# harrisonvanderbyl/rwkv-cpp-accelerated

Measured on AMD Instinct MI355X. Metric: tokens/sec single-stream RWKV-4 uint8 greedy decode, higher is better.
Workload: dtype u8 weights x 23-bit fixed-point activations, exact 32-bit integer accumulate (tile form: v_mfma_i32_16x16x64_i8 on signed limbs; row form: v_dot4_u32_u8 on the VALU); f32/f64 epilogues, f64 state; 1 GPU; RWKV-4-Raven-7B uint8 single-stream greedy decode (L=32, D=4096, V=50277), 32-token prompt then 1885-token continuation, device-resident state; parallelism=1 GPU

## Files before the change

rwkv-cpp-accelerated_amd/csrc/engine.hip:

```cpp
#include "kernels.hip.h"
#include "tile.hip.h"
#include "seq.hip.h"
#include "sampler.hip.h"
#include "../../include/rwkv_mi355x.h"

#include <dlfcn.h>

#include <algorithm>
#include <atomic>
#include <chrono>
#include <unistd.h>
#include <cstdarg>
#include <cstdio>
#include <cstdlib>
#include <cstring>
#include <map>
#include <string>
#include <tuple>
#include <vector>

using namespace rwkvk;

namespace {

// ... 127 lines not shown
    int seq_rows = SEQ_TM;
    int seq_b = -1;
    int tile = -1;

    float *embed = nullptr;
    double *ln = nullptr, *mixk = nullptr, *mixv = nullptr, *mixr = nullptr, *fmixk = nullptr, *fmixr = nullptr;
    float *kr = nullptr, *vr = nullptr, *rr = nullptr, *o1 = nullptr, *o2 = nullptr, *o3 = nullptr;
    float *attr = nullptr, *atto = nullptr, *fkr = nullptr, *fvr = nullptr, *frr = nullptr;
    float *fko = nullptr, *fvo = nullptr, *fro = nullptr, *headr = nullptr, *heado = nullptr;
    double *uw = nullptr, *ew = nullptr;
    float *siteC[3] = {nullptr, nullptr, nullptr};
    float *siteP[3] = {nullptr, nullptr, nullptr};
    double *siteTC[3] = {nullptr, nullptr, nullptr};
    float *siteMC[3] = {nullptr, nullptr, nullptr};
    float *siteB[3] = {nullptr, nullptr, nullptr};
    double *sitePD[3] = {nullptr, nullptr, nullptr};
    float *sitePF[3] = {nullptr, nullptr, nullptr};
    double *lnstat = nullptr;
    uint8_t *w_kvr = nullptr, *w_att = nullptr, *w_frk = nullptr, *w_fv = nullptr, *w_head = nullptr;
    unsigned *rs_kvr = nullptr, *rs_att = nullptr, *rs_frk = nullptr, *rs_fv = nullptr, *rs_head = nullptr;
    double *state[5] = {nullptr, nullptr, nullptr, nullptr, nullptr};
    double *x = nullptr, *partA = nullptr, *partF = nullptr;
    float *ybuf = nullptr, *hbuf = nullptr, *rgate = nullptr, *logits = nullptr, *blk_val = nullptr, *partMA = nullptr, *partMF = nullptr;
    unsigned *blk_idx = nullptr;
    Ctl *ctl = nullptr;
    Ctl *h_ctl = nullptr;
    unsigned long long *gen = nullptr;
    unsigned long long *pick = nullptr;
    double *ts_part = nullptr;
    float *ts_p = nullptr, *ts_pw = nullptr;
    unsigned *ts_key = nullptr;
    unsigned gen_cap = 0;
    hipGraphExec_t g_fwd = nullptr, g_greedy = nullptr;
    unsigned *herr = nullptr, *d_herr = nullptr;
    unsigned long long *tl = nullptr;
    bool tl_on = false;
    int tl_cls = 3;
    bool seq_ok = false;
    unsigned long long *sq_tokens = nullptr;
    unsigned long long *h_sq_tokens = nullptr;
    hipEvent_t sq_ev[8] = {};
    uint64_t sq_n = 0;
    struct SeqGraphKey { uint64_t la, lb, row0; int buf, n; bool operator<(const SeqGraphKey &o) const { return std::tie(la, lb, row0, buf, n) < std::tie(o.la, o.lb, o.row0, o.buf, o.n); } };
    std::map<SeqGraphKey, hipGraphExec_t> sq_graphs;
    bool seq_graph = true;
    int graphs = 3;
    double *sq_x[4] = {nullptr, nullptr, nullptr, nullptr};
    hipEvent_t xs_ev[2] = {nullptr, nullptr};
    static constexpr int SPLIT_MAX = 4;
    int n_split = 0;
    hipStream_t sp_stream[SPLIT_MAX] = {};
    struct SeqScratch *sp_scratch[SPLIT_MAX] = {};
    hipEvent_t sp_done[SPLIT_MAX][SPLIT_MAX] = {};
    hipEvent_t sp_end = nullptr;
    double *x_in = nullptr;
    struct Pipe *pipe = nullptr;
    bool pipe_prof = false;
    static constexpr size_t HOP_EV = 512;
    hipEvent_t hop_ev[2 * HOP_EV] = {};
    double hop_stats[4] = {0.0, 0.0, 0.0, 0.0};
    Ctl *pipe_ring = nullptr;
    uint64_t pipe_ring_cap = 0;
    double *sq_state = nullptr;
    float *sq_y = nullptr;
    unsigned *sq_img[3] = {nullptr, nullptr, nullptr}, *sq_imgh = nullptr;
    SeqPart *sq_qpart = nullptr, *sq_qparta = nullptr, *sq_qparth = nullptr;
// ... 86 lines not shown
    HIPCHK(hipFuncSetAttribute(reinterpret_cast<const void *>(kernel), hipFuncAttributeMaxDynamicSharedMemorySize, (int)bytes));
    return 0;
}


struct ArgMaker {
    rwkv_ctx *c;
    int D, grid, n_first;
    size_t LD;
    explicit ArgMaker(rwkv_ctx *c_) : c(c_), D((int)c_->D), grid(c_->grid), LD((size_t)c_->L * c_->D) { n_first = grid < 32 ? grid : 32; }
    unsigned long long *tl_of(int k, uint64_t l) const { return (c->tl_on && k == c->tl_cls && l == (c->l0 + c->l1) / 2) ? c->tl : nullptr; }
    SiteStatic site_static(int k, uint64_t ll) const
    {
        const int nv = SITE_NV[k], pw = SITE_PW[k];
        SiteStatic st;
        st.C = c->siteC[k] + (size_t)ll * nv * D; st.P = c->siteP[k] + (size_t)ll * D * pw;
        st.TC = c->siteTC[k] + (size_t)ll * nv; st.maxC = c->siteMC[k] + (size_t)ll * nv;
        st.invD = 1.0 / (double)D; st.invDm1 = 1.0 / (double)(D - 1);
        return st;
    }
    SiteDyn site_dyn(int k, int n_part) const
    {
        SiteDyn dy;
        dy.B = c->siteB[k]; dy.pd = c->sitePD[k]; dy.pf = c->sitePF[k]; dy.lnstat = c->lnstat + 2 * k; dy.n_part = n_part;
        return dy;
    }
    FirstArgs first() const
    {
        FirstArgs fa;
        fa.embed = c->embed; fa.ln = c->ln; fa.x = c->x; fa.x_in = c->x_in ? c->x_in : c->x; fa.st = site_static(0, c->l0); fa.dy = site_dyn(0, n_first);
        fa.sxy = c->state[0] + (size_t)c->l0 * D; fa.slot_stride = LD; fa.ctl = c->ctl; fa.D = D; fa.from_token = c->l0 == 0;
        return fa;
    }
    AttArgs att(uint64_t l) const
    {
        const size_t lo = (size_t)l * D;
        AttArgs aa;
        aa.x = c->x; aa.st = site_static(0, l); aa.dy = site_dyn(0, l == c->l0 ? n_first : grid);
        aa.w = c->w_kvr ? c->w_kvr + (size_t)(l - c->l0) * 3 * D * D : nullptr; aa.rs = c->rs_kvr + (size_t)(l - c->l0) * D * 3;
        aa.uw = c->uw + lo; aa.ew = c->ew + lo;
        aa.r_att = c->attr + lo; aa.o_att = c->atto + lo;
        aa.saa = c->state[1] + lo; aa.sbb = c->state[2] + lo;
        aa.slot_stride = LD; aa.ybuf = c->ybuf; aa.partS = c->partA; aa.partM = c->partMA;
        aa.ctl = c->ctl; aa.D = D; aa.ns = 0; aa.tl = tl_of(1, l); aa.herr = c->d_herr;
        return aa;
    }
    AttOutArgs attout(uint64_t l) const
    {
        const size_t lo = (size_t)l * D;
        AttOutArgs ao;
        ao.w = c->w_att ? c->w_att + (size_t)(l - c->l0) * D * D : nullptr; ao.rs = c->rs_att + (size_t)(l - c->l0) * D; ao.ybuf = c->ybuf; ao.partS = c->partA; ao.partM = c->partMA; ao.n_part = grid;
        ao.x = c->x; ao.lnw = c->ln + (4 * l + 2) * D; ao.lnb = c->ln + (4 * l + 3) * D; ao.lnstat = c->lnstat + 0;
        ao.sxy = c->state[0] + lo; ao.st = site_static(1, l); ao.dy = site_dyn(1, grid); ao.sdd = c->state[4] + lo;
        ao.slot_stride = LD; ao.ctl = c->ctl; ao.D = D; ao.ns = 0; ao.tl = tl_of(2, l); ao.herr = c->d_herr;
        return ao;
    }
    FfnRKArgs frk(uint64_t l) const
    {
        const size_t lo = (size_t)l * D;
        FfnRKArgs fa;
        fa.x = c->x; fa.st = site_static(1, l); fa.dy = site_dyn(1, grid);
        fa.w = c->w_frk ? c->w_frk + (size_t)(l - c->l0) * 5 * D * D : nullptr; fa.rs = c->rs_frk + (size_t)(l - c->l0) * D * 5;
        fa.r_fv = c->fvr + 4 * lo; fa.o_fv = c->fvo + 4 * lo;
        fa.hbuf = c->hbuf; fa.rgate = c->rgate; fa.partS = c->partF; fa.partM = c->partMF; fa.ctl = c->ctl; fa.D = D;
        fa.ns = 0; fa.tl = tl_of(3, l); fa.herr = c->d_herr;
        return fa;
// ... 63 lines not shown
            ta.im.CB = mk.D / c->tile_th; ta.im.bimg = c->t_frk + (size_t)(l - c->l0) * 5 * (size_t)mk.D * mk.D;
            const size_t sm = tile_smem(c, 3);
            TILE_DISPATCH(c, (k_ffn_rk_t<4, 4, 64, 16, 1><<<dim3(grid), dim3(NT), sm, c->stream>>>(ta)),
                          (k_ffn_rk_t<5, 5, 20, 4, 5><<<dim3(grid), dim3(NT), sm, c->stream>>>(ta)),
                          (k_ffn_rk_t<2, 4, 8, 4, 2><<<dim3(grid), dim3(NT), sm, c->stream>>>(ta)));
        }
        else DISPATCH_S(S, k_ffn_rk<S_><<<dim3(grid), dim3(NT), smem_frk(S), c->stream>>>(fa));
    } break;
    case 4: {
        FfnVArgs fv = mk.fv(l);
        if (tile_ok(c, 4)) {
            FfnVTArgs ta;
            ta.a = fv; ta.a.ns = tile_units(c, 4);
            ta.im.CB = mk.D / c->tile_th; ta.im.bimg = c->t_fv + (size_t)(l - c->l0) * 4 * (size_t)mk.D * mk.D;
            const size_t sm = tile_smem(c, 4);
            if (mk.fv_next_att(l))
                TILE_DISPATCH(c, (k_ffnv_t<4, 4, 256, 16, 1, 3><<<dim3(grid), dim3(NT), sm, c->stream>>>(ta)),
                              (k_ffnv_t<5, 5, 80, 4, 5, 3><<<dim3(grid), dim3(NT), sm, c->stream>>>(ta)),
                              (k_ffnv_t<2, 4, 32, 4, 2, 3><<<dim3(grid), dim3(NT), sm, c->stream>>>(ta)));
            else
                TILE_DISPATCH(c, (k_ffnv_t<4, 4, 256, 16, 1, 1><<<dim3(grid), dim3(NT), sm, c->stream>>>(ta)),
                              (k_ffnv_t<5, 5, 80, 4, 5, 1><<<dim3(grid), dim3(NT), sm, c->stream>>>(ta)),
                              (k_ffnv_t<2, 4, 32, 4, 2, 1><<<dim3(grid), dim3(NT), sm, c->stream>>>(ta)));
        }
        else if (mk.fv_next_att(l)) {
            DISPATCH_S(S, k_ffnv<S_, 3><<<dim3(grid), dim3(NT), smem_fv(S), c->stream>>>(fv));
        } else {
            DISPATCH_S(S, k_ffnv<S_, 1><<<dim3(grid), dim3(NT), smem_fv(S), c->stream>>>(fv));
        }
    } break;
    case 5: {
        HeadArgs ha = mk.head();
        DISPATCH_S(S, k_head<S_><<<dim3(grid), dim3(NT), smem_head(S), c->stream>>>(ha));
    } break;
    default:
        k_argmax_finish<<<dim3(1), dim3(64), 0, c->stream>>>(c->blk_val, c->blk_idx, grid, c->ctl, c->gen, c->gen_cap);
    }
}

int device_check(rwkv_ctx *c)
{
    if (!c->herr || *c->herr == 0u) return 0;
    const unsigned code = *c->herr;
    *c->herr = 0u;
    return fail(RWKV_E_DEVICE, "a device-side wait gave up (code %u: an LDS hand-off timed out; is the GPU shared or preempted?) -- "
                               "the results of this call are invalid; RWKV_TILE=0 selects kernels without bounded waits", code);
}

int enqueue_token(rwkv_ctx *c, bool with_argmax, hipEvent_t *ev)
{
    const bool last = c->l1 == c->L;
    int evi = 0;
#define EV() do { if (ev) HIPCHK(hipEventRecord(ev[evi++], c->stream)); } while (0)
    EV();
    launch_class(c, 0, 0);
    for (uint64_t l = c->l0; l < c->l1; l++)
        for (int cls = 1; cls <= 4; cls++) { EV(); launch_class(c, cls, l); }
    EV();
    if (last) launch_class(c, 5, 0);
    EV();
    if (last && with_argmax) launch_class(c, 6, 0);
    EV();
#undef EV
    HIPCHK(hipGetLastError());
    return 0;
}

int build_graph(rwkv_ctx *c, bool with_argmax, hipGraphExec_t *out)
{
    hipGraph_t g = nullptr;
    HIPCHK(hipStreamBeginCapture(c->stream, hipStreamCaptureModeRelaxed));
    int rc = enqueue_token(c, with_argmax, nullptr);
    hipError_t e = hipStreamEndCapture(c->stream, &g);
    if (rc) return rc;
    HIPCHK(e);
    HIPCHK(hipGraphInstantiate(out, g, nullptr, nullptr, 0));
    HIPCHK(hipGraphDestroy(g));
    return 0;
}

int rebuild_graphs(rwkv_ctx *c)
{
    int rc = 0;
    if (c->g_fwd) { (void)hipGraphExecDestroy(c->g_fwd); c->g_fwd = nullptr; rc = build_graph(c, false, &c->g_fwd); if (rc) { c->g_fwd = nullptr; return rc; } }
    if (c->g_greedy) { (void)hipGraphExecDestroy(c->g_greedy); c->g_greedy = nullptr; rc = build_graph(c, true, &c->g_greedy); if (rc) { c->g_greedy = nullptr; return rc; } }
    return 0;
}

int retile(rwkv_ctx *c, Source &src, int slot, uint64_t layer, uint64_t N, uint64_t M, uint8_t *dst,
           int G, int RS, int off, uint8_t *staging)
{
    const uint8_t *dsrc = static_cast<const uint8_t *>(src.device_ptr(slot, layer * N * M));
    if (!dsrc) {
        int rc = src.to_device(slot, layer * N * M, N * M, staging, c->stream);
        if (rc) return rc;
        dsrc = staging;
    }
    dim3 grid((unsigned)((M + 63) / 64), (unsigned)((N + 63) / 64));
    hipLaunchKernelGGL(k_retile, grid, dim3(256), 0, c->stream, dsrc, dst, (int)N, (int)M, G, RS, off);
    HIPCHK(hipGetLastError());
    return 0;
}

template <typename T> int upload(rwkv_ctx *c, Source &src, int slot, T **dst)
{
    const uint64_t n = tensor_elems(slot, c->L, c->D);
    int rc = dalloc(c, dst, n);
    if (rc) return rc;
    return src.to_device(slot, 0, n * sizeof(T), *dst, c->stream);
}

int seq_smem_limits()
{
    int rc = 0;
#define SEQ_ALLOW_P(TAG, NTW, NKB, NVS, DEPTH, MULTI) if (!rc) rc = allow_smem(k_seq_gemm_p<TAG, NTW, NKB, NVS, DEPTH, MULTI>, seq_gemm_p_smem(NKB, NVS, MULTI))
    SEQ_ALLOW_P(0, 3, 8, 3, RWKV_SEQ_DEPTH0, false); SEQ_ALLOW_P(0, 3, 10, 2, 2, false);
    SEQ_ALLOW_P(1, 1, 8, 1, 8, false); SEQ_ALLOW_P(1, 1, 10, 1, 10, false);
    SEQ_ALLOW_P(2, 5, 8, 2, RWKV_SEQ_DEPTH2, false); SEQ_ALLOW_P(2, 4, 10, 2, 2, false);
// ... 260 lines not shown
            if ((rc = dalloc(c, &c->sq_tokens, (size_t)SQ_RING * SEQ_TM))) return rc;
            HIPCHK(hipHostMalloc(reinterpret_cast<void **>(&c->h_sq_tokens), sizeof(unsigned long long) * SQ_RING * SEQ_TM, hipHostMallocDefault));
            for (int r = 0; r < SQ_RING; r++) HIPCHK(hipEventCreateWithFlags(&c->sq_ev[r], hipEventDisableTiming));
            if ((rc = dalloc(c, &c->sq_x[0], (size_t)SEQ_TM * D))) return rc;
            if ((rc = dalloc(c, &c->sq_x[1], (size_t)SEQ_TM * D))) return rc;
            if ((rc = dalloc(c, &c->sq_state, (size_t)D))) return rc;
            if ((rc = dalloc(c, &c->sq_y, (size_t)SEQ_TM * D))) return rc;
            for (int k = 0; k < 3; k++) {
                if ((rc = dalloc(c, &c->sq_img[k], 2 * a_image_bytes(D) / 4))) return rc;
                HIPCHK(hipMemsetAsync(c->sq_img[k], 0, 2 * a_image_bytes(D), c->stream));
            }
            if ((rc = dalloc(c, &c->sq_imgh, 2 * a_image_bytes(4 * D) / 4))) return rc;
            HIPCHK(hipMemsetAsync(c->sq_imgh, 0, 2 * a_image_bytes(4 * D), c->stream));
            if ((rc = dalloc(c, &c->sq_qpart, (size_t)2 * 3 * SEQ_T * SEQ_O))) return rc;
            if ((rc = dalloc(c, &c->sq_qparta, (size_t)2 * SEQ_T * SEQ_O))) return rc;
            if ((rc = dalloc(c, &c->sq_qparth, (size_t)2 * SEQ_T * SEQ_O))) return rc;
            HIPCHK(hipMemsetAsync(c->sq_qpart, 0, sizeof(SeqPart) * 2 * 3 * SEQ_T * SEQ_O, c->stream));
            HIPCHK(hipMemsetAsync(c->sq_qparta, 0, sizeof(SeqPart) * 2 * SEQ_T * SEQ_O, c->stream));
            HIPCHK(hipMemsetAsync(c->sq_qparth, 0, sizeof(SeqPart) * 2 * SEQ_T * SEQ_O, c->stream));
            if ((rc = dalloc(c, &c->sq_stat, (size_t)SEQ_TM * SEQ_O))) return rc;
            {
                const size_t cbd = ((size_t)D + 15) / 16;
                if ((rc = dalloc(c, &c->sq_pk3, (size_t)2 * SEQ_O * 3 * cbd * 512))) return rc;
                if ((rc = dalloc(c, &c->sq_pk5, (size_t)2 * SEQ_O * 5 * cbd * 512))) return rc;
                if ((rc = dalloc(c, &c->sq_pk1, (size_t)2 * SEQ_O * cbd * 512))) return rc;
            }
            c->seq_ok = true;
        }
    }
    HIPCHK(hipStreamSynchronize(c->stream));
    if ((rc = set_smem_limits(c))) return rc;
    if (c->seq_ok && (rc = seq_smem_limits())) return rc;
    if (c->graphs & 1) {
        if ((rc = build_graph(c, false, &c->g_fwd))) return rc;
        if ((rc = build_graph(c, true, &c->g_greedy))) return rc;
    }
    c->loaded = true;
    return 0;
}

struct ChunkPart { uint64_t la, lb; hipStream_t st; const SeqScratch *S; bool no_upload = false; const unsigned long long *dtok = nullptr; };
int upload_chunk_tokens(rwkv_ctx *c, const uint64_t *tokens, int n, int buf, hipStream_t st)
{
    const int slot = (int)(c->sq_n % SQ_RING);
    if (c->sq_n >= SQ_RING) HIPCHK(hipEventSynchronize(c->sq_ev[slot]));
    unsigned long long *h = c->h_sq_tokens + (size_t)slot * SEQ_TM, *d = c->sq_tokens + (size_t)buf * SEQ_TM;
    for (int t = 0; t < n; t++) h[t] = tokens[t];
    HIPCHK(hipMemcpyAsync(d, h, sizeof(unsigned long long) * n, hipMemcpyHostToDevice, st));
    HIPCHK(hipEventRecord(c->sq_ev[slot], st));
    c->sq_n++;
    return 0;
}
int enqueue_chunk(rwkv_ctx *c, const uint64_t *tokens, int n, uint64_t row0, bool par, int buf = 0, const ChunkPart *part = nullptr)
{
    const int D = (int)c->D;
    const uint64_t L = c->L, V = RWKV_VOCAB;
    const uint64_t la = part ? part->la : c->l0, lb = part ? part->lb : c->l1;
    const bool first = c->l0 == 0 && la == c->l0, last = c->l1 == c->L && lb == c->l1;
    hipStream_t st = part ? part->st : c->stream;
    SeqScratch own;
    own.state = c->sq_state; own.y = c->sq_y; own.imgh = c->sq_imgh;
    for (int k = 0; k < 3; k++) own.img[k] = c->sq_img[k];
    own.qpart = c->sq_qpart; own.qparta = c->sq_qparta; own.qparth = c->sq_qparth; own.stat = c->sq_stat;
    own.pk3 = c->sq_pk3; own.pk5 = c->sq_pk5; own.pk1 = c->sq_pk1;
    const SeqScratch &S = part ? *part->S : own;
    double *x = c->sq_x[buf];
    if (first) {
        if (buf < 0 || buf >= SQ_RING) return fail(RWKV_E_ARG, "residual buffer %d out of range", buf);
// ... 286 lines not shown
                const uint64_t *tk = (k == 0 && tokens) ? tokens + t0 : nullptr;
                if (mode == RWKV_MODE_PARRALEL) rc = enqueue_chunk(c, tk, n, t0, true, b, &part);
                else rc = enqueue_pass(c, tk, n, t0, b, part);
                HIPCHK(hipEventRecord(c->sp_done[k][b], st));
            }
        }
        for (int k = 1; k < ns; k++) {
            HIPCHK(hipEventRecord(c->sp_end, c->sp_stream[k]));
            HIPCHK(hipStreamWaitEvent(c->stream, c->sp_end, 0));
        }
        return rc;
    }
    if (rc) return rc;
    for (uint64_t t0 = 0; t0 < T; t0 += CH) {
        const int n = (int)(T - t0 < CH ? T - t0 : CH);
        ChunkPart part{c->l0, c->l1, c->stream, &own};
        if (dtok) part.dtok = dtok + t0;
        if (mode == RWKV_MODE_PARRALEL) rc = enqueue_chunk(c, tokens ? tokens + t0 : nullptr, n, t0, true, 0, &part);
        else rc = enqueue_pass(c, tokens + t0, n, t0, 0, part);
        if (rc) return rc;
    }
    return 0;
}

int begin_call(rwkv_ctx *c)
{
    if (c->herr) *c->herr = 0u;
    return 0;
}

int run_token(rwkv_ctx *c, bool with_argmax)
{
    hipGraphExec_t g = with_argmax ? c->g_greedy : c->g_fwd;
    if (g) { HIPCHK(hipGraphLaunch(g, c->stream)); return 0; }
    return enqueue_token(c, with_argmax, nullptr);
}

const struct { const char *name, *instead; } RETIRED_ENV[] = {
    {"RWKV_RING", "RWKV_TILE (the LDS-ring form of the row-form decode kernels is gone)"},
    {"RWKV_NO_GRAPH", "RWKV_GRAPH=0"},
    {"RWKV_SEQ_GRAPH", "RWKV_GRAPH bit 1"},
    {"RWKV_SEQ_SPLIT", "RWKV_SEQ_STAGES (RWKV_SEQ_SPLIT=0 is RWKV_SEQ_STAGES=1)"},
    {"RWKV_PIPE_LOG", nullptr},
    {"RWKV_SEQ_PIPE", nullptr},
    {"RWKV_SEQ_SMALL", nullptr},
};
void warn_retired_env()
{
    for (const auto &r : RETIRED_ENV)
        if (getenv(r.name))
            fprintf(stderr, "[rwkv_mi355x] %s is retired and ignored%s%s\n", r.name, r.instead ? "; use " : "", r.instead ? r.instead : "");
}

}

extern "C" {

const char *rwkv_last_error(void) { return g_err.c_str(); }

int rwkv_create(rwkv_ctx **out, int device)
{
    if (!out) return fail(RWKV_E_ARG, "out is NULL");
    int n = 0;
    if (hipGetDeviceCount(&n) != hipSuccess || n <= 0)
        return fail(RWKV_E_DEVICE, "no HIP device available (this engine has no CPU fallback)");
    if (device < 0 || device >= n) return fail(RWKV_E_ARG, "device %d out of range (have %d)", device, n);
    HIPCHK(hipSetDevice(device));
// ... 140 lines not shown
    if (T > c->maxT) return fail(RWKV_E_ARG, "n_tokens %llu > max context %llu", (unsigned long long)T, (unsigned long long)c->maxT);
    double *h[5] = {xy, aa, bb, pp, dd};
    HIPCHK(hipSetDevice(c->device));
    if (logits) HIPCHK(hipMemcpyAsync(logits, c->logits, T * RWKV_VOCAB * sizeof(float), hipMemcpyDeviceToHost, c->stream));
    const size_t bytes = T * c->L * c->D * sizeof(double);
    for (int s = 0; s < 5; s++)
        if (h[s]) HIPCHK(hipMemcpyAsync(h[s], c->state[s], bytes, hipMemcpyDeviceToHost, c->stream));
    HIPCHK(hipStreamSynchronize(c->stream));
    return device_check(c);
}

int rwkv_reset_state(rwkv_ctx *c)
{
    if (!c) return fail(RWKV_E_ARG, "NULL ctx");
    if (!c->loaded) return fail(RWKV_E_STATE, "RWKV not loaded");
    HIPCHK(hipSetDevice(c->device));
    for (int s = 0; s < 5; s++)
        HIPCHK(hipMemsetAsync(c->state[s], 0, c->maxT * c->L * c->D * sizeof(double), c->stream));
    HIPCHK(hipStreamSynchronize(c->stream));
    return device_check(c);
}

int rwkv_decode_greedy(rwkv_ctx *c, uint64_t first_token, uint64_t n, uint64_t *out_tokens)
{
    if (!c || !out_tokens) return fail(RWKV_E_ARG, "NULL argument");
    if (!c->loaded) return fail(RWKV_E_STATE, "RWKV not loaded");
    if (c->l0 != 0 || c->l1 != c->L) return fail(RWKV_E_STATE, "needs a whole-model context (a pipeline stage has no embedding / head of its own)");
    if (first_token >= RWKV_VOCAB) return fail(RWKV_E_ARG, "token id out of range");
    if (n == 0 || n > c->gen_cap) return fail(RWKV_E_ARG, "n_tokens must be in 1..%u", c->gen_cap);
    HIPCHK(hipSetDevice(c->device));
    { const int rcp = begin_call(c); if (rcp) return rcp; }
    c->h_ctl[0].token = first_token; c->h_ctl[0].slot = 0; c->h_ctl[0].out_row = 0; c->h_ctl[0].step = 0; c->h_ctl[0].pad = 0;
    HIPCHK(hipMemcpyAsync(c->ctl, &c->h_ctl[0], sizeof(Ctl), hipMemcpyHostToDevice, c->stream));
    for (uint64_t i = 0; i < n; i++) {
        int rc = run_token(c, true);
        if (rc) return rc;
    }
    HIPCHK(hipMemcpyAsync(out_tokens, c->gen, n * sizeof(uint64_t), hipMemcpyDeviceToHost, c->stream));
    HIPCHK(hipStreamSynchronize(c->stream));
    return device_check(c);
}

namespace {
TypicalArgs typical_args(rwkv_ctx *c, float temp, float tau, int flags)
{
    TypicalArgs a{};
    a.recipe = (flags & RWKV_SAMPLE_RECIPE) ? 1 : 0;
    if (a.recipe) a.expo = temp == 1.0f ? 1.0 : 1.0 / (double)temp;
    else { const double e = 1.0 / (double)temp; a.expo = temp == 1.0f ? 1.0 : (e >= 255.0 ? 255.0 : (double)(unsigned char)e); }
    a.logits = c->logits; a.ctl = c->ctl; a.gen = c->gen; a.gen_cap = c->gen_cap;
    a.temp = temp; a.tau = tau; a.ban0 = (flags & RWKV_SAMPLE_BAN0) ? 1 : 0; a.step = -1; a.seeds = nullptr;
    a.pick = c->pick; a.part = c->ts_part; a.p = c->ts_p; a.pw = c->ts_pw; a.key = c->ts_key;
    return a;
}
int enqueue_typical(rwkv_ctx *c, const TypicalArgs &a, unsigned rows)
{
    k_typical_stats<<<dim3(TS_G, rows), dim3(TS_GT), 0, c->stream>>>(a);
    k_typical_keys<<<dim3(TS_G, rows), dim3(TS_GT), 0, c->stream>>>(a);
    k_typical<<<dim3(1, rows), dim3(TS_NT), 0, c->stream>>>(a);
    HIPCHK(hipGetLastError());
    return 0;
}
int launch_typical(rwkv_ctx *c, int row, float temp, float tau, double u, uint64_t seed, bool use_seed, int flags, bool feedback)
{
    TypicalArgs a = typical_args(c, temp, tau, flags);
    a.row = row; a.u = u; a.seed = seed; a.use_seed = use_seed ? 1 : 0; a.feedback = feedback ? 1 : 0;
    return enqueue_typical(c, a, 1);
}
}

// ... 114 lines not shown
int rwkv_decode_batch_greedy(rwkv_ctx *c, const uint64_t *first_tokens, uint64_t n_streams, uint64_t n_steps, uint64_t *out_tokens)
{
    return decode_batch(c, first_tokens, n_streams, n_steps, false, 1.0f, 0.0f, nullptr, 0, out_tokens);
}

int rwkv_decode_batch_typical(rwkv_ctx *c, const uint64_t *first_tokens, uint64_t n_streams, uint64_t n_steps, float temp, float tau,
                              const uint64_t *seeds, int flags, uint64_t *out_tokens)
{
    return decode_batch(c, first_tokens, n_streams, n_steps, true, temp, tau, seeds, flags, out_tokens);
}

int rwkv_state_copy(rwkv_ctx *c, uint64_t dst, uint64_t src)
{
    if (!c) return fail(RWKV_E_ARG, "NULL ctx");
    if (!c->loaded) return fail(RWKV_E_STATE, "RWKV not loaded");
    if (dst >= c->maxT || src >= c->maxT)
        return fail(RWKV_E_ARG, "state slot out of range (dst %llu, src %llu, max context %llu)", (unsigned long long)dst, (unsigned long long)src, (unsigned long long)c->maxT);
    if (dst == src) return 0;
    const size_t n = (size_t)c->L * c->D;
    HIPCHK(hipSetDevice(c->device));
    for (int s = 0; s < 5; s++)
        HIPCHK(hipMemcpyAsync(c->state[s] + dst * n, c->state[s] + src * n, n * sizeof(double), hipMemcpyDeviceToDevice, c->stream));
    HIPCHK(hipStreamSynchronize(c->stream));
    return device_check(c);
}

void rwkv_free(rwkv_ctx *c)
{
    if (!c) return;
    (void)hipSetDevice(c->device);
    if (c->stream) (void)hipStreamSynchronize(c->stream);
    if (c->g_fwd) { (void)hipGraphExecDestroy(c->g_fwd); c->g_fwd = nullptr; }
    if (c->g_greedy) { (void)hipGraphExecDestroy(c->g_greedy); c->g_greedy = nullptr; }
    rwkv_pipe_free(c);
    for (void *p : c->allocs) (void)hipFree(p);
    for (rwkv_ctx::Grown *g : {&c->bd_ids, &c->bd_val, &c->bd_idx, &c->bd_part, &c->bd_p, &c->bd_pw, &c->bd_key}) if (g->p) (void)hipFree(g->p);
    if (c->h_ctl) (void)hipHostFree(c->h_ctl);
    if (c->herr) (void)hipHostFree(c->herr);
    for (auto &e : c->xs_ev) if (e) (void)hipEventDestroy(e);
    for (auto &e : c->hop_ev) if (e) (void)hipEventDestroy(e);
    for (auto &row : c->sp_done) for (auto &e : row) if (e) (void)hipEventDestroy(e);
    if (c->sp_end) (void)hipEventDestroy(c->sp_end);
    for (int k = 1; k < rwkv_ctx::SPLIT_MAX; k++) { if (c->sp_stream[k]) (void)hipStreamDestroy(c->sp_stream[k]); delete c->sp_scratch[k]; }
    for (auto &kv : c->sq_graphs) (void)hipGraphExecDestroy(kv.second);
    c->sq_graphs.clear();
    if (c->h_sq_tokens) (void)hipHostFree(c->h_sq_tokens);
    for (int r = 0; r < SQ_RING; r++) if (c->sq_ev[r]) (void)hipEventDestroy(c->sq_ev[r]);
    if (c->stream) (void)hipStreamDestroy(c->stream);
    delete c;
}

float *rwkv_logits_device(rwkv_ctx *c) { return c ? c->logits : nullptr; }
double *rwkv_state_device(rwkv_ctx *c, int which) { return (c && which >= 0 && which < 5) ? c->state[which] : nullptr; }
void *rwkv_stream(rwkv_ctx *c) { return c ? (void *)c->stream : nullptr; }
int rwkv_abi_version(void) { return RWKV_MI355X_ABI_VERSION; }
uint64_t rwkv_resident_bytes(const rwkv_ctx *c) { return c ? (uint64_t)c->alloc_bytes : 0; }
int rwkv_decode_form(const rwkv_ctx *c) { return c && c->loaded ? (c->tile > 0 ? c->tile : 0) : -1; }

uint64_t rwkv_bytes_per_token(const rwkv_ctx *c)
{
    if (!c) return 0;
    const uint64_t nl = (c->l1 == UINT64_MAX ? c->L : c->l1) - c->l0, D = c->D, V = RWKV_VOCAB;
    return 13 * nl * D * D + (c->l1 == c->L || c->l1 == UINT64_MAX ? V * D : 0) + 168 * nl * D + 40 * D;
}

int rwkv_profile_token(rwkv_ctx *c, uint64_t token, int reps, double *ms, uint64_t *bytes, uint32_t *launches)
// ... 87 lines not shown
{
    if (!c || !out) return fail(RWKV_E_ARG, "NULL argument");
    if (!c->loaded) return fail(RWKV_E_STATE, "RWKV not loaded");
    const size_t n = (size_t)(c->grid > 512 ? c->grid : 512) * NW * 8;
    if (cap < n) return fail(RWKV_E_ARG, "need room for %zu stamps", n);
    HIPCHK(hipSetDevice(c->device));
    { const int rcp = begin_call(c); if (rcp) return rcp; }
    if (!c->tl) { int rc = dalloc(c, &c->tl, n); if (rc) return rc; }
    HIPCHK(hipMemsetAsync(c->tl, 0, n * 8, c->stream));
    c->h_ctl[0].token = token; c->h_ctl[0].slot = 0; c->h_ctl[0].out_row = 0; c->h_ctl[0].step = 0; c->h_ctl[0].pad = 0;
    HIPCHK(hipMemcpyAsync(c->ctl, &c->h_ctl[0], sizeof(Ctl), hipMemcpyHostToDevice, c->stream));
    { const char *e = getenv("RWKV_TL_CLASS"); c->tl_cls = e ? atoi(e) : 3; }
    c->tl_on = true;
    int rc;
    if (c->tl_cls >= 10) {
        if (!c->seq_ok) { c->tl_on = false; return fail(RWKV_E_STATE, "the chunk path is not loaded (max_ctx 1)"); }
        uint64_t toks[SEQ_TM];
        for (int t = 0; t < SEQ_TM; t++) toks[t] = token;
        int rows = SEQ_T;
        if (c->tl_cls >= 20) { c->tl_cls -= 10; if (c->seq_rows > SEQ_T && c->maxT >= (uint64_t)SEQ_TM) rows = SEQ_TM; }
        rc = enqueue_chunk(c, toks, rows, 0, false);
    } else rc = enqueue_token(c, false, nullptr);
    c->tl_on = false;
    if (rc) return rc;
    HIPCHK(hipMemcpyAsync(out, c->tl, n * 8, hipMemcpyDeviceToHost, c->stream));
    HIPCHK(hipStreamSynchronize(c->stream));
    return device_check(c);
}

int rwkv_debug_launch(rwkv_ctx *c, int cls, uint64_t layer, uint64_t token, uint32_t slot)
{
    if (!c) return fail(RWKV_E_ARG, "NULL ctx");
    if (!c->loaded) return fail(RWKV_E_STATE, "RWKV not loaded");
    if (cls < 0 || cls > 6) return fail(RWKV_E_ARG, "kernel class %d out of range (0 first, 1 att, 2 att_out, 3 ffn r+k, 4 ffn_v, 5 head, 6 argmax)", cls);
    if (cls >= 1 && cls <= 4 && (layer < c->l0 || layer >= c->l1)) return fail(RWKV_E_ARG, "layer %llu is not one of this context's", (unsigned long long)layer);
    if (cls >= 5 && c->l1 != c->L) return fail(RWKV_E_STATE, "this context does not hold the head");
    if (slot >= c->maxT) return fail(RWKV_E_ARG, "state slot %u out of range", slot);
    if (c->l0 == 0 && token >= RWKV_VOCAB) return fail(RWKV_E_ARG, "token id out of range");
    HIPCHK(hipSetDevice(c->device));
    { const int rcp = begin_call(c); if (rcp) return rcp; }
    if (cls == 0) {
        c->h_ctl[0].token = token; c->h_ctl[0].slot = slot; c->h_ctl[0].out_row = slot; c->h_ctl[0].step = 0; c->h_ctl[0].pad = 0;
        HIPCHK(hipMemcpyAsync(c->ctl, &c->h_ctl[0], sizeof(Ctl), hipMemcpyHostToDevice, c->stream));
    }
    launch_class(c, cls, layer);
    HIPCHK(hipGetLastError());
    HIPCHK(hipStreamSynchronize(c->stream));
    return device_check(c);
}

namespace {
int debug_buf(rwkv_ctx *c, int which, void **p, size_t *bytes)
{
    const size_t D = (size_t)c->D, G = (size_t)c->grid;
    switch (which) {
    case RWKV_DBG_X: *p = c->x; *bytes = D * 8; break;
    case RWKV_DBG_YBUF: *p = c->ybuf; *bytes = D * 4; break;
    case RWKV_DBG_PART_ATT: *p = c->partA; *bytes = G * 8; break;
    case RWKV_DBG_PMAX_ATT: *p = c->partMA; *bytes = G * 4; break;
    case RWKV_DBG_HBUF: *p = c->hbuf; *bytes = 4 * D * 4; break;
    case RWKV_DBG_RGATE: *p = c->rgate; *bytes = D * 4; break;
    case RWKV_DBG_PART_FFN: *p = c->partF; *bytes = G * 8; break;
    case RWKV_DBG_PMAX_FFN: *p = c->partMF; *bytes = G * 4; break;
    case RWKV_DBG_LNSTAT: *p = c->lnstat; *bytes = 6 * 8; break;
    default: return fail(RWKV_E_ARG, "no such debug buffer: %d", which);
    }
    return 0;
}
}
// ... 587 lines not shown
```

rwkv-cpp-accelerated_amd/csrc/kernels.hip.h:

```cpp
#pragma once
#include <hip/hip_runtime.h>
#include <stdint.h>

namespace rwkvk {

constexpr int NT = 512;
constexpr int NW = NT / 64;
constexpr int RED_BYTES = 1024;
#define RWKV_ARGS_NOW(...) asm volatile("" ::RWKV_ARGS_S(__VA_ARGS__))
#define RWKV_ARGS_S(...) RWKV_ARGS_PICK(__VA_ARGS__, RWKV_A8, RWKV_A7, RWKV_A6, RWKV_A5, RWKV_A4, RWKV_A3, RWKV_A2, RWKV_A1)(__VA_ARGS__)
#define RWKV_ARGS_PICK(a, b, c, d, e, f, g, h, N, ...) N
#define RWKV_A1(a) "s"(a)
#define RWKV_A2(a, ...) "s"(a), RWKV_A1(__VA_ARGS__)
#define RWKV_A3(a, ...) "s"(a), RWKV_A2(__VA_ARGS__)
#define RWKV_A4(a, ...) "s"(a), RWKV_A3(__VA_ARGS__)
#define RWKV_A5(a, ...) "s"(a), RWKV_A4(__VA_ARGS__)
#define RWKV_A6(a, ...) "s"(a), RWKV_A5(__VA_ARGS__)
#define RWKV_A7(a, ...) "s"(a), RWKV_A6(__VA_ARGS__)
#define RWKV_A8(a, ...) "s"(a), RWKV_A7(__VA_ARGS__)
__device__ __forceinline__ int wave_id() { return __builtin_amdgcn_readfirstlane((int)(threadIdx.x >> 6)); }
__device__ __forceinline__ int block_lo(int n) { return (int)(((unsigned)blockIdx.x * (unsigned)n) / gridDim.x); }
__device__ __forceinline__ int block_hi(int n) { return (int)((((unsigned)blockIdx.x + 1u) * (unsigned)n) / gridDim.x); }
constexpr unsigned VOCAB = 50277u;
constexpr float QLIM = 4194000.0f;
// ... 604 lines not shown
    fail = ok ? fail : 3u;
}
__device__ __forceinline__ void ring_report(unsigned fail, unsigned *herr)
{
    if (fail != 0u && herr != nullptr && (threadIdx.x & 63) == 0) __hip_atomic_store(herr, fail, __ATOMIC_RELAXED, __HIP_MEMORY_SCOPE_SYSTEM);
}
#ifndef RWKV_RING_DEPTH
#define RWKV_RING_DEPTH 28
#endif
#ifndef RWKV_RING_PRE
#define RWKV_RING_PRE 8
#endif
#ifndef RWKV_TEST_DROP_GROUP
#define RWKV_TEST_DROP_GROUP 0
#endif
#ifndef RWKV_RING_PRE_DEPTH
#define RWKV_RING_PRE_DEPTH 20
#endif
constexpr int NC = NW - 1;

struct FirstArgs {
    const float *embed;
    const double *ln;
    double *x;
    const double *x_in;
    SiteStatic st;
    SiteDyn dy;
    const double *sxy;
    size_t slot_stride;
    const Ctl *ctl;
    int D;
    int from_token;
};
__global__ __launch_bounds__(NT) void k_first(FirstArgs a)
{
    __shared__ double red[RED_BYTES / 8];
    const int D = a.D;
    const int j0 = block_lo(D), j1 = block_hi(D);
    const size_t so = (size_t)a.ctl->slot * a.slot_stride;
    double mean = 0.0, rstd = 1.0;
    const float *row = a.from_token ? a.embed + (size_t)a.ctl->token * D : nullptr;
    if (a.from_token) {
        double s[2] = {0.0, 0.0};
        for (int j = threadIdx.x; j < D; j += NT) { const double v = (double)row[j]; s[0] += v; s[1] += v * v; }
        block_sum<2>(s, red + RED_STATS);
        mean = s[0] / (double)D;
        rstd = 1.0 / sqrt((s[1] - s[0] * mean) / (double)(D - 1));
        __syncthreads();
    }
    SiteAcc<3> acc;
    acc.clear();
    for (int j = j0 + threadIdx.x; j < j1; j += NT) {
        double x;
        if (a.from_token) { x = a.ln[j] * (((double)row[j] - mean) * rstd) + a.ln[D + j]; a.x[j] = x; }
        else { x = a.x_in[j]; a.x[j] = x; }
        SitePre<3> pre;
        site_prefetch<3>(a.st, j, pre);
        site_emit<3>(pre, a.dy, D, j, x, a.sxy[so + j], acc);
    }
    site_publish<3, 64>(acc, a.dy, red);
}

struct AttArgs {
    const double *x;
    SiteStatic st;
    SiteDyn dy;
    const uint8_t *w;
    const unsigned *rs;
    const double *uw, *ew;
    const float *r_att, *o_att;
    double *saa, *sbb;
    size_t slot_stride;
    float *ybuf;
    double *partS;
    float *partM;
    const Ctl *ctl;
    int D;
    int ns;
    unsigned long long *tl;
    unsigned *herr;
};

__device__ __forceinline__ void att_epilogue(double *saa, double *sbb, float *ybuf, int g, double aa, double bb, double e1, double ek, float v, float r, double ew, float ra, float oa, double &part, float &pmax)
{
    const double vv = (double)v;
    double y = (aa + e1 * vv) / (bb + e1);
    y = (1.0 / (1.0 + (double)expf(-r))) * y;
    saa[g] = (aa + ek * vv) * ew;
    sbb[g] = (bb + ek) * ew;
    const float yf = (float)y;
    const float ys = yf * ra;
    ybuf[g] = ys;
    part += (double)(yf * oa);
    pmax = fmaxf(pmax, fabsf(ys));
// ... 280 lines not shown
        site_prefetch<NVN>(a.st, g, in.pre);
        return in;
    };
    auto epi = [&](int g, const unsigned long long (&T)[4], const FfnVIn<NVN> &in) {
        if (lane == 0)
            ffnv_epilogue<NVN>(a, so, D, g, row_value((T[0] + T[1]) + (T[2] + T[3]), in.rsum, sc) + Sf, in.rg, in.xold, in.lw, in.lb, in.prevn, mean2, rstd2, in.pre, acc);
    };
    u32x4 wA[4][S];
    int gA;
    unsigned *gctr = group_counter(red);
    first_groups(g0, wave, gctr, gA);
    vec_open<4, 4, S, (RWKV_SPLIT & 8) != 0>(a.hbuf, a.partS, a.partM, a.n_part, D, red, xq, wA, base(gA), (size_t)D, Sf, amax, a.tl);
    sc = scale_of(amax);
    stream_groups<4, S, PAT_PER_ROW>(wA, gA, g0, g1, gctr, xq, lane, (size_t)D, chunks, base, pre, epi);
    __syncthreads();
    tl_stamp(a.tl, 6);
    site_publish<NVN, 1>(acc, a.dy, xq);
    tl_stamp(a.tl, 7);
}

struct HeadArgs {
    const double *x;
    SiteStatic st;
    SiteDyn dy;
    const uint8_t *w;
    const unsigned *rs;
    float *logits;
    float *blk_val;
    unsigned *blk_idx;
    const Ctl *ctl;
    int D;
};

__device__ __forceinline__ bool am_better(float v, unsigned i, float best, unsigned besti) { return v > best || (v == best && i < besti); }
__device__ __forceinline__ void am_wave_fold(float &best, unsigned &besti)
{
#pragma unroll
    for (int m = 32; m >= 1; m >>= 1) {
        const float ov = __shfl_xor(best, m, 64);
        const unsigned oi = __shfl_xor(besti, m, 64);
        if (am_better(ov, oi, best, besti)) { best = ov; besti = oi; }
    }
}

template <int R> struct HeadIn { unsigned rsr[R]; int row0, shift; };
template <int S, int R = RWKV_HEAD_R>
__global__ __launch_bounds__(NT) void k_head(HeadArgs a)
{
    extern __shared__ __attribute__((aligned(16))) unsigned char smem[];
    constexpr int XVD = xvd<S>();
    double *red = reinterpret_cast<double *>(smem);
    unsigned *xq = reinterpret_cast<unsigned *>(smem + RED_BYTES);
    float *bval = reinterpret_cast<float *>(xq + XVD);
    unsigned *bidx = reinterpret_cast<unsigned *>(bval + NW);
    const int D = a.D, lane = threadIdx.x & 63, wave = wave_id();
    const int chunks = D >> 4;
    const int V = (int)VOCAB;
    const int G = (V + R - 1) / R;
    const int g0 = block_lo(G);
    const int g1 = block_hi(G);
    float *lg = a.logits + (size_t)a.ctl->out_row * V;

    auto base = [&](int gg) {
        int row = (gg < g1 ? gg : (g1 > g0 ? g1 - 1 : 0)) * R;
        if (row > V - R) row = V - R;
        return a.w + (size_t)row * D;
    };
    float Sf;
    double sc;
    float best = -INFINITY;
    unsigned besti = 0xffffffffu;
    auto pre = [&](int g) {
        HeadIn<R> in;
        in.row0 = g * R;
        in.shift = (in.row0 > V - R) ? in.row0 - (V - R) : 0;
        in.row0 -= in.shift;
#pragma unroll
// ... 166 lines not shown
```

Before: 634.1 tokens/s.

## Fuse greedy argmax finish into next token's first kernel via turn graph

Adds a k_turn kernel that performs the final argmax over head block partials inside every block, then immediately loads the chosen embedding row and runs the first-layer LayerNorm and site emission. The greedy loop now launches a 'turn' graph (layers, head, turn) per token, which removes the separate single-block k_argmax_finish launch and its serialization before the next token's k_first. It also restructures first_body to prefetch embedding, LN weights, state and site inputs into registers up front, assuming one element per thread per block. The cost is redundant per-block argmax work and a stricter assumption on grid and width sizes.

```diff
diff --git a/rwkv-cpp-accelerated_amd/csrc/engine.hip b/rwkv-cpp-accelerated_amd/csrc/engine.hip
--- a/rwkv-cpp-accelerated_amd/csrc/engine.hip
+++ b/rwkv-cpp-accelerated_amd/csrc/engine.hip
@@ -183,6 +183,8 @@
     unsigned *ts_key = nullptr;
     unsigned gen_cap = 0;
     hipGraphExec_t g_fwd = nullptr, g_greedy = nullptr;
+    hipGraphExec_t g_turn = nullptr;
+    bool head_ran = false;
     unsigned *herr = nullptr, *d_herr = nullptr;
     unsigned long long *tl = nullptr;
     bool tl_on = false;
@@ -335,6 +337,13 @@
         fa.sxy = c->state[0] + (size_t)c->l0 * D; fa.slot_stride = LD; fa.ctl = c->ctl; fa.D = D; fa.from_token = c->l0 == 0;
         return fa;
     }
+    TurnArgs turn() const
+    {
+        TurnArgs ta;
+        ta.f = first();
+        ta.p.blk_val = c->blk_val; ta.p.blk_idx = c->blk_idx; ta.p.n_blk = grid; ta.p.gen_cap = c->gen_cap; ta.p.ctl = c->ctl; ta.p.gen = c->gen;
+        return ta;
+    }
     AttArgs att(uint64_t l) const
     {
         const size_t lo = (size_t)l * D;
@@ -464,9 +473,15 @@
     case 5: {
         HeadArgs ha = mk.head();
         DISPATCH_S(S, k_head<S_><<<dim3(grid), dim3(NT), smem_head(S), c->stream>>>(ha));
+        c->head_ran = true;
     } break;
-    default:
+    case 6:
         k_argmax_finish<<<dim3(1), dim3(64), 0, c->stream>>>(c->blk_val, c->blk_idx, grid, c->ctl, c->gen, c->gen_cap);
+        break;
+    default: {
+        TurnArgs ta = mk.turn();
+        k_turn<<<dim3(mk.n_first), dim3(NT), 0, c->stream>>>(ta);
+    }
     }
 }
 
@@ -498,12 +513,25 @@
     return 0;
 }
 
-int build_graph(rwkv_ctx *c, bool with_argmax, hipGraphExec_t *out)
+int enqueue_turn(rwkv_ctx *c)
+{
+    for (uint64_t l = c->l0; l < c->l1; l++)
+        for (int cls = 1; cls <= 4; cls++) launch_class(c, cls, l);
+    launch_class(c, 5, 0);
+    launch_class(c, 7, 0);
+    HIPCHK(hipGetLastError());
+    return 0;
+}
+
+enum TokenGraph { TG_FWD, TG_PICK, TG_TURN };
+int build_graph(rwkv_ctx *c, TokenGraph kind, hipGraphExec_t *out)
 {
     hipGraph_t g = nullptr;
+    const bool head_ran = c->head_ran;
     HIPCHK(hipStreamBeginCapture(c->stream, hipStreamCaptureModeRelaxed));
-    int rc = enqueue_token(c, with_argmax, nullptr);
+    int rc = kind == TG_TURN ? enqueue_turn(c) : enqueue_token(c, kind == TG_PICK, nullptr);
     hipError_t e = hipStreamEndCapture(c->stream, &g);
+    c->head_ran = head_ran;
     if (rc) return rc;
     HIPCHK(e);
     HIPCHK(hipGraphInstantiate(out, g, nullptr, nullptr, 0));
@@ -514,8 +542,9 @@
 int rebuild_graphs(rwkv_ctx *c)
 {
     int rc = 0;
-    if (c->g_fwd) { (void)hipGraphExecDestroy(c->g_fwd); c->g_fwd = nullptr; rc = build_graph(c, false, &c->g_fwd); if (rc) { c->g_fwd = nullptr; return rc; } }
-    if (c->g_greedy) { (void)hipGraphExecDestroy(c->g_greedy); c->g_greedy = nullptr; rc = build_graph(c, true, &c->g_greedy); if (rc) { c->g_greedy = nullptr; return rc; } }
+    if (c->g_fwd) { (void)hipGraphExecDestroy(c->g_fwd); c->g_fwd = nullptr; rc = build_graph(c, TG_FWD, &c->g_fwd); if (rc) { c->g_fwd = nullptr; return rc; } }
+    if (c->g_greedy) { (void)hipGraphExecDestroy(c->g_greedy); c->g_greedy = nullptr; rc = build_graph(c, TG_PICK, &c->g_greedy); if (rc) { c->g_greedy = nullptr; return rc; } }
+    if (c->g_turn) { (void)hipGraphExecDestroy(c->g_turn); c->g_turn = nullptr; rc = build_graph(c, TG_TURN, &c->g_turn); if (rc) { c->g_turn = nullptr; return rc; } }
     return 0;
 }
 
@@ -842,8 +871,9 @@
     if ((rc = set_smem_limits(c))) return rc;
     if (c->seq_ok && (rc = seq_smem_limits())) return rc;
     if (c->graphs & 1) {
-        if ((rc = build_graph(c, false, &c->g_fwd))) return rc;
-        if ((rc = build_graph(c, true, &c->g_greedy))) return rc;
+        if ((rc = build_graph(c, TG_FWD, &c->g_fwd))) return rc;
+        if ((rc = build_graph(c, TG_PICK, &c->g_greedy))) return rc;
+        if (first && last && (rc = build_graph(c, TG_TURN, &c->g_turn))) return rc;
     }
     c->loaded = true;
     return 0;
@@ -1196,7 +1226,7 @@
 int run_token(rwkv_ctx *c, bool with_argmax)
 {
     hipGraphExec_t g = with_argmax ? c->g_greedy : c->g_fwd;
-    if (g) { HIPCHK(hipGraphLaunch(g, c->stream)); return 0; }
+    if (g) { HIPCHK(hipGraphLaunch(g, c->stream)); c->head_ran = c->head_ran || c->l1 == c->L; return 0; }
     return enqueue_token(c, with_argmax, nullptr);
 }
 
@@ -1403,10 +1433,12 @@
     { const int rcp = begin_call(c); if (rcp) return rcp; }
     c->h_ctl[0].token = first_token; c->h_ctl[0].slot = 0; c->h_ctl[0].out_row = 0; c->h_ctl[0].step = 0; c->h_ctl[0].pad = 0;
     HIPCHK(hipMemcpyAsync(c->ctl, &c->h_ctl[0], sizeof(Ctl), hipMemcpyHostToDevice, c->stream));
+    launch_class(c, 0, 0);
     for (uint64_t i = 0; i < n; i++) {
-        int rc = run_token(c, true);
-        if (rc) return rc;
-    }
+        if (c->g_turn) { HIPCHK(hipGraphLaunch(c->g_turn, c->stream)); c->head_ran = true; }
+        else { const int rc = enqueue_turn(c); if (rc) return rc; }
+    }
+    HIPCHK(hipGetLastError());
     HIPCHK(hipMemcpyAsync(out_tokens, c->gen, n * sizeof(uint64_t), hipMemcpyDeviceToHost, c->stream));
     HIPCHK(hipStreamSynchronize(c->stream));
     return device_check(c);
@@ -1587,6 +1619,7 @@
     if (c->stream) (void)hipStreamSynchronize(c->stream);
     if (c->g_fwd) { (void)hipGraphExecDestroy(c->g_fwd); c->g_fwd = nullptr; }
     if (c->g_greedy) { (void)hipGraphExecDestroy(c->g_greedy); c->g_greedy = nullptr; }
+    if (c->g_turn) { (void)hipGraphExecDestroy(c->g_turn); c->g_turn = nullptr; }
     rwkv_pipe_free(c);
     for (void *p : c->allocs) (void)hipFree(p);
     for (rwkv_ctx::Grown *g : {&c->bd_ids, &c->bd_val, &c->bd_idx, &c->bd_part, &c->bd_p, &c->bd_pw, &c->bd_key}) if (g->p) (void)hipFree(g->p);
@@ -1740,9 +1773,11 @@
 {
     if (!c) return fail(RWKV_E_ARG, "NULL ctx");
     if (!c->loaded) return fail(RWKV_E_STATE, "RWKV not loaded");
-    if (cls < 0 || cls > 6) return fail(RWKV_E_ARG, "kernel class %d out of range (0 first, 1 att, 2 att_out, 3 ffn r+k, 4 ffn_v, 5 head, 6 argmax)", cls);
+    if (cls < 0 || cls > 7) return fail(RWKV_E_ARG, "kernel class %d out of range (0 first, 1 att, 2 att_out, 3 ffn r+k, 4 ffn_v, 5 head, 6 argmax, 7 turn)", cls);
     if (cls >= 1 && cls <= 4 && (layer < c->l0 || layer >= c->l1)) return fail(RWKV_E_ARG, "layer %llu is not one of this context's", (unsigned long long)layer);
     if (cls >= 5 && c->l1 != c->L) return fail(RWKV_E_STATE, "this context does not hold the head");
+    if (cls == 7 && c->l0 != 0) return fail(RWKV_E_STATE, "this context does not hold the embedding");
+    if (cls == 7 && !c->head_ran) return fail(RWKV_E_STATE, "kernel class 7 picks from the head's partials, and this context has not launched a head yet");
     if (slot >= c->maxT) return fail(RWKV_E_ARG, "state slot %u out of range", slot);
     if (c->l0 == 0 && token >= RWKV_VOCAB) return fail(RWKV_E_ARG, "token id out of range");
     HIPCHK(hipSetDevice(c->device));
diff --git a/rwkv-cpp-accelerated_amd/csrc/kernels.hip.h b/rwkv-cpp-accelerated_amd/csrc/kernels.hip.h
--- a/rwkv-cpp-accelerated_amd/csrc/kernels.hip.h
+++ b/rwkv-cpp-accelerated_amd/csrc/kernels.hip.h
@@ -660,17 +660,95 @@
     int D;
     int from_token;
 };
-__global__ __launch_bounds__(NT) void k_first(FirstArgs a)
+__device__ __forceinline__ bool am_better(float v, unsigned i, float best, unsigned besti) { return v > best || (v == best && i < besti); }
+__device__ __forceinline__ void am_wave_fold(float &best, unsigned &besti)
+{
+#pragma unroll
+    for (int m = 32; m >= 1; m >>= 1) {
+        const float ov = __shfl_xor(best, m, 64);
+        const unsigned oi = __shfl_xor(besti, m, 64);
+        if (am_better(ov, oi, best, besti)) { best = ov; besti = oi; }
+    }
+}
+struct PickArgs {
+    const float *blk_val;
+    const unsigned *blk_idx;
+    int n_blk;
+    unsigned gen_cap;
+    Ctl *ctl;
+    unsigned long long *gen;
+};
+constexpr int FIRST_K = 10;
+constexpr int PICK_K = 4;
+static_assert(FIRST_K * NT >= 5120 && PICK_K * 64 >= NT / 2, "first_body's register batches cover the widest model and the largest grid");
+
+template <bool PICK>
+__device__ __forceinline__ void first_body(const FirstArgs &a, const PickArgs &p)
 {
     __shared__ double red[RED_BYTES / 8];
-    const int D = a.D;
+    __shared__ unsigned picked;
+    const unsigned slot = a.ctl->slot;
+    const unsigned long long token0 = PICK ? 0ull : a.ctl->token;
+    RWKV_ARGS_NOW(a.ln, a.st.P, a.sxy, a.slot_stride, a.D, a.embed, a.from_token);
+    if (PICK) RWKV_ARGS_NOW(p.blk_val, p.blk_idx, p.n_blk);
+    const int D = a.D, tid = threadIdx.x, lane = tid & 63, wave = wave_id();
+    const bool ft = PICK || a.from_token;
     const int j0 = block_lo(D), j1 = block_hi(D);
-    const size_t so = (size_t)a.ctl->slot * a.slot_stride;
+    const int j = j0 + tid, jc = j < D ? j : D - 1;
+    float rv[FIRST_K], xr = 0.f;
+    auto row_request = [&](unsigned long long token) {
+        const float *row = a.embed + (size_t)token * D;
+#pragma unroll
+        for (int k = 0; k < FIRST_K; k++) { const int jj = tid + k * NT; rv[k] = row[jj < D ? jj : D - 1]; }
+        xr = row[jc];
+    };
+    float pv[PICK_K];
+    unsigned pi[PICK_K];
+    if (PICK && wave == 0) {
+#pragma unroll
+        for (int k = 0; k < PICK_K; k++) {
+            const int i = lane + 64 * k, ic = i < p.n_blk ? i : p.n_blk - 1;
+            pv[k] = p.blk_val[ic]; pi[k] = p.blk_idx[ic];
+        }
+    }
+    double lnw = 0.0, lnb = 0.0, xin = 0.0;
+    if (ft) { lnw = a.ln[jc]; lnb = a.ln[D + jc]; }
+    else xin = a.x_in[jc];
+    SitePre<3> pre;
+    site_prefetch<3>(a.st, jc, pre);
+    __builtin_amdgcn_sched_barrier(0);
+    if (!PICK) RWKV_ARGS_NOW(token0);
+    const double prev = a.sxy[(size_t)slot * a.slot_stride + jc];
+    __builtin_amdgcn_sched_barrier(0);
+    if (!PICK && ft) row_request(token0);
+    __builtin_amdgcn_sched_barrier(0);
+    if (PICK) {
+        if (wave == 0) {
+            float best = -INFINITY;
+            unsigned besti = 0xffffffffu;
+#pragma unroll
+            for (int k = 0; k < PICK_K; k++)
+                if (lane + 64 * k < p.n_blk && am_better(pv[k], pi[k], best, besti)) { best = pv[k]; besti = pi[k]; }
+            am_wave_fold(best, besti);
+            if (lane == 0) picked = besti >= VOCAB ? 0u : besti;
+        }
+        __syncthreads();
+        const unsigned id = picked;
+        row_request(id);
+        if (blockIdx.x == 0 && tid == 0) {
+            const unsigned step = p.ctl->step;
+            if (step < p.gen_cap) p.gen[step] = id;
+            p.ctl->token = id;
+            p.ctl->step = step + 1;
+        }
+        __builtin_amdgcn_sched_barrier(0);
+    }
     double mean = 0.0, rstd = 1.0;
-    const float *row = a.from_token ? a.embed + (size_t)a.ctl->token * D : nullptr;
-    if (a.from_token) {
+    if (ft) {
         double s[2] = {0.0, 0.0};
-        for (int j = threadIdx.x; j < D; j += NT) { const double v = (double)row[j]; s[0] += v; s[1] += v * v; }
+#pragma unroll
+        for (int k = 0; k < FIRST_K; k++)
+            if (tid + k * NT < D) { const double v = (double)rv[k]; s[0] += v; s[1] += v * v; }
         block_sum<2>(s, red + RED_STATS);
         mean = s[0] / (double)D;
         rstd = 1.0 / sqrt((s[1] - s[0] * mean) / (double)(D - 1));
@@ -678,16 +756,17 @@
     }
     SiteAcc<3> acc;
     acc.clear();
-    for (int j = j0 + threadIdx.x; j < j1; j += NT) {
+    if (j < j1) {
         double x;
-        if (a.from_token) { x = a.ln[j] * (((double)row[j] - mean) * rstd) + a.ln[D + j]; a.x[j] = x; }
-        else { x = a.x_in[j]; a.x[j] = x; }
-        SitePre<3> pre;
-        site_prefetch<3>(a.st, j, pre);
-        site_emit<3>(pre, a.dy, D, j, x, a.sxy[so + j], acc);
+        if (ft) { x = lnw * (((double)xr - mean) * rstd) + lnb; a.x[j] = x; }
+        else { x = xin; a.x[j] = x; }
+        site_emit<3>(pre, a.dy, D, j, x, prev, acc);
     }
     site_publish<3, 64>(acc, a.dy, red);
 }
+__global__ __launch_bounds__(NT) void k_first(FirstArgs a) { first_body<false>(a, PickArgs{}); }
+struct TurnArgs { FirstArgs f; PickArgs p; };
+__global__ __launch_bounds__(NT) void k_turn(TurnArgs a) { first_body<true>(a.f, a.p); }
 
 struct AttArgs {
     const double *x;
@@ -1034,17 +1113,6 @@
     int D;
 };
 
-__device__ __forceinline__ bool am_better(float v, unsigned i, float best, unsigned besti) { return v > best || (v == best && i < besti); }
-__device__ __forceinline__ void am_wave_fold(float &best, unsigned &besti)
-{
-#pragma unroll
-    for (int m = 32; m >= 1; m >>= 1) {
-        const float ov = __shfl_xor(best, m, 64);
-        const unsigned oi = __shfl_xor(besti, m, 64);
-        if (am_better(ov, oi, best, besti)) { best = ov; besti = oi; }
-    }
-}
-
 template <int R> struct HeadIn { unsigned rsr[R]; int row0, shift; };
 template <int S, int R = RWKV_HEAD_R>
 __global__ __launch_bounds__(NT) void k_head(HeadArgs a)
```

Result: no change. 635.3 tokens/s, median of 6 (+0.2%).
